# toandaominh1997/EfficientDet.Pytorch

Measured on AMD Instinct MI355X. Metric: images/sec EfficientDet-D0 512px fwd+bwd, higher is better.
Workload: dtype f32_hf16x3_bwd_bf16x3

## Files before the change

efficientdet/pytorch_amd/_lib.py:

```python
import ctypes as C
import os

import torch

HERE = os.path.dirname(os.path.abspath(__file__))
LIB_PATH = os.environ.get('EFFDET_HIP_LIB') or os.path.join(os.path.dirname(os.path.abspath(__file__)), 'libeffdet_hip.so')
MAX_SEG = 5
MAX_CONV_SEG = 10
ABI_VERSION = 11
F32, BF16, F32_BF16X3, F32_SPLIT = 0, 1, 2, 3
F32_HSPLIT = 4
ACT_NONE, ACT_RELU, ACT_SWISH, ACT_SIGMOID = 0, 1, 2, 3
RES_NONE, RES_ADD, RES_RELU_MASK, RES_SWISH_GRAD = 0, 1, 2, 3
TUNE_IGEMM_BIG, TUNE_IGEMM_BIG_MIN_M, TUNE_SPLIT_PERS, TUNE_IGEMM_KORD, TUNE_SPLIT_KORD = 0, 1, 2, 3, 4

_ERR = {-1: 'EFFDET_EINVAL', -2: 'EFFDET_ELAUNCH', -3: 'EFFDET_EUNSUPPORTED'}


class Seg(C.Structure):
    _fields_ = [('H', C.c_int), ('W', C.c_int), ('Ho', C.c_int), ('Wo', C.c_int),
                ('in_off', C.c_longlong), ('in_bstride', C.c_longlong),
                ('out_off', C.c_longlong), ('out_bstride', C.c_longlong)]


# ... 200 lines not shown
}
EMA_SIGNATURES = {
    'effdet_clip_adamw_step_ema': 'i:ppppppppiippffffffifipps',
    'effdet_clip_adamw_step_gated_ema': 'i:pppppppppiippfffffffippps',
    'effdet_ema_swap': 'i:pppppiis',
}
PLAN_SIGNATURES = {
    'effdet_dwconv_plan_info': 'i:iiiiiiiiiiiiip',
}
LIVE_SIGNATURES = {
    'effdet_live_tiles_counts': 'q:iipppp',
    'effdet_live_tiles': 'i:piiiippppps',
    'effdet_conv2d_live': 'i:ppis',
    'effdet_conv2d_wgrad_live': 'i:ppqps',
}
BOX_LOSS_SIGNATURES = {
    'effdet_box_loss_fwd': 'i:ppppppqiqiiifs',
    'effdet_box_loss_fwd_grad': 'i:ppppppqpiiiqiiifs',
    'effdet_box_loss_bwd_reg': 'i:ppppppiiiqiifs',
}
LOSS_OPTS_SIGNATURES = {
    'effdet_loss_opts_workspace_bytes': 'q:iqii',
    'effdet_loss_opts_fwd': 'i:ppppppqiqiips',
    'effdet_loss_opts_fwd_grad': 'i:ppppppqpiiiqiips',
    'effdet_loss_opts_bwd_cls': 'i:pppppiiiqiips',
    'effdet_loss_opts_bwd_reg': 'i:ppppppiiiqips',
}
ATSS_SIGNATURES = {
    'effdet_loss_atss_workspace_bytes': 'q:iqiip',
    'effdet_loss_atss_fwd': 'i:ppppppqiqiipps',
# ... 16 lines not shown
    global _lib
    if _lib is None:
        if not os.path.exists(LIB_PATH):
            raise RuntimeError(
                'libeffdet_hip.so is missing (%s). Build it with `python -m efficientdet.pytorch_amd.build` '
                '(or __graft_entry__.build()). There is no CPU fallback for this path.' % LIB_PATH)
        cand = C.CDLL(LIB_PATH)
        got = int(cand.effdet_abi_version()) if hasattr(cand, 'effdet_abi_version') else 0
        if got != ABI_VERSION:
            raise RuntimeError('%s has ABI generation %d, this binding needs %d: rebuild it (`python -m efficientdet.pytorch_amd.build`)'
                               % (LIB_PATH, got, ABI_VERSION))
        _lib = cand
        for name, sig in list(SIGNATURES.items()) + list(ADDED_SIGNATURES.items()) + list(EMA_SIGNATURES.items()) + \
                list(PLAN_SIGNATURES.items()) + list(LIVE_SIGNATURES.items()) + list(BOX_LOSS_SIGNATURES.items()) + \
                list(LOSS_OPTS_SIGNATURES.items()) + list(ATSS_SIGNATURES.items()) + list(CONV_PLAN_SIGNATURES.items()) + \
                list(WBF_SIGNATURES.items()):
            f = getattr(_lib, name, None)
            if f is not None:
                f.restype, f.argtypes = _CTYPE[sig[0]], [_CTYPE[c] for c in sig[2:]]
    return _lib


def require(*names):
    L = lib()
    missing = [n for n in names if not hasattr(L, n)]
    if missing:
        raise RuntimeError('%s does not export %s: it predates this binding, rebuild it (`python -m efficientdet.pytorch_amd.build`)'
                           % (LIB_PATH, ', '.join(missing)))
    return L


# ... 25 lines not shown
```

efficientdet/pytorch_amd/csrc/conv_igemm.hip:

```cpp
#include "common.h"
#include "../../../include/effdet_live_tiles.h"
#include "../../../include/effdet_conv_plan.h"
#include <stdlib.h>

#ifndef EFFDET_IGEMM_BIG_DEFAULT
#define EFFDET_IGEMM_BIG_DEFAULT 1
#endif

namespace {

struct SegD {
  int H, W, Ho, Wo, M, tile_start;
  long long in_off, in_bs, out_off, out_bs;
  unsigned x_bytes;
  long long w_off;
  long long sh_off;
};

struct ConvK {
  const void* x; const void* w; void* y; void* z; const void* res;
  const float* scale; const float* shift; const float* rowscale;
  const float* bc_scale; const float* bc_shift;
  int Cin, Cout, KW, stride, pad_t, pad_l;
  int ldx, ldy;
  int Kc;
  int cpt;
  int act, res_mode, out_f32, vec_ok;
  int out_split;
  int* range_flag;
  void* ysplit;
  int nseg, mtiles, ntiles;
  unsigned w_bytes;
  int kord;
  long long w_img_bytes;
  const unsigned char* live;
  int live_tile0;
  SegD seg[EFFDET_MAX_CONV_SEG];
};

constexpr int BM = 128;
typedef float f32x16 __attribute__((ext_vector_type(16)));

template <typename T> struct Mma;
template <> struct Mma<bf16_t> {
  static __device__ __forceinline__ void run(const uint4& a, const uint4& b, f32x4& c) {
    c = __builtin_amdgcn_mfma_f32_16x16x32_bf16(__builtin_bit_cast(bf16x8, a), __builtin_bit_cast(bf16x8, b), c, 0, 0, 0);
  }
};
struct MmaH {
  static __device__ __forceinline__ void run(const uint4& a, const uint4& b, f32x4& c) {
    c = __builtin_amdgcn_mfma_f32_16x16x32_f16(__builtin_bit_cast(f16x8, a), __builtin_bit_cast(f16x8, b), c, 0, 0, 0);
// ... 31 lines not shown

  const int tid = threadIdx.x;
  const int lane = tid & 63, wave = tid >> 6;
  const int wm0 = (wave / WAVES_N) * WTM, wn0 = (wave % WAVES_N) * WTN;

  int tile = xcd_remap(blockIdx.x, gridDim.x);
  if constexpr (SPLIT == 2) {
    if (p.live) {
      const int b = blockIdx.x, whole = (p.mtiles >> 3) << 3;
      if (b < whole * p.ntiles) {
        const int i = b >> 3, j = i / p.ntiles;
        tile = (j * 8 + (b & 7)) * p.ntiles + (i - j * p.ntiles);
      } else tile = b;
    }
  }
  const int mt = tile / p.ntiles, nt = tile - mt * p.ntiles;
  int si = 0;
#pragma unroll
  for (int s = 1; s < EFFDET_MAX_CONV_SEG; ++s)
    if (s < p.nseg && mt >= p.seg[s].tile_start) si = s;
  const SegD sg = p.seg[si];
  const int m_base = (mt - sg.tile_start) * BM;
  const int n_base = nt * BN;
  const int HoWo = sg.Ho * sg.Wo;

  if constexpr (SPLIT == 2) {
    if (p.live && mt >= p.live_tile0 && p.live[mt - p.live_tile0] == 0) {
      if (p.res_mode == EFFDET_RES_ADD) return;
      const int rows = min(BM, sg.M - m_base), nch = min(BN, p.Cout - n_base);
      if (p.vec_ok) {
        const int q4 = nch >> 2;
        for (int i = tid; i < rows * q4; i += NTHREADS) {
          const int row = i / q4, c = i - row * q4;
          const int m = m_base + row, bi = m / HoWo, pix = m - bi * HoWo;
          *(uint4*)((float*)p.y + sg.out_off + (long long)bi * sg.out_bs + (long long)pix * p.ldy + n_base + 4 * c) = make_uint4(0u, 0u, 0u, 0u);
        }
      } else {
        for (int i = tid; i < rows * nch; i += NTHREADS) {
          const int row = i / nch, c = i - row * nch;
          const int m = m_base + row, bi = m / HoWo, pix = m - bi * HoWo;
          ((float*)p.y)[sg.out_off + (long long)bi * sg.out_bs + (long long)pix * p.ldy + n_base + c] = 0.f;
        }
      }
      return;
    }
  }

  constexpr unsigned ES = sizeof(T);
  const long long w_img = p.w_img_bytes ? (long long)(m_base / HoWo) * p.w_img_bytes : 0ll;
  const u32x4_t rx = make_srd_raw((const T*)p.x + sg.in_off, sg.x_bytes), rw = make_srd_raw((const char*)p.w + w_img + sg.w_off, p.w_bytes);
// ... 1032 lines not shown
  k.bc_scale = p->bc_scale; k.bc_shift = p->bc_shift;
  if ((p->bc_scale != nullptr) != (p->bc_shift != nullptr)) return EFFDET_EINVAL;
  k.Cin = p->Cin; k.Cout = p->Cout; k.KW = p->KW; k.stride = p->stride; k.pad_t = p->pad_t; k.pad_l = p->pad_l;
  k.ldx = p->ldx; k.ldy = p->ldy;
  k.cpt = p->Cin / ce; k.Kc = p->KH * p->KW * k.cpt;
  k.act = p->act; k.res_mode = p->res_mode; k.out_f32 = p->out_f32; k.kord = g_tuning[EFFDET_TUNE_IGEMM_KORD];
  k.out_split = (splitfmt && !p->out_f32) ? 1 : 0;
  if (splitfmt) {
    if (g_tuning[EFFDET_TUNE_SPLIT_KORD] < 0) g_tuning[EFFDET_TUNE_SPLIT_KORD] = getenv("EFFDET_SPLIT_KORD") ? atoi(getenv("EFFDET_SPLIT_KORD")) : 1;
    const int kv = g_tuning[EFFDET_TUNE_SPLIT_KORD];
    k.kord = ((kv == 1 || (kv == 2 && p->Cout <= 64)) && k.cpt % 8 == 0) ? 1 : 0;
  }
  k.nseg = p->nseg;
  k.w_img_bytes = p->w_image_stride;
  k.live = nullptr; k.live_tile0 = 0;
  if (p->w_image_stride) {
    if (p->w_image_stride < 0 || (p->w_image_stride & 15) || p->nseg != 1 || splitfmt || (p->seg[0].Ho * p->seg[0].Wo) % BM) return EFFDET_EUNSUPPORTED;
  }
  int tiles = 0;
  bool per_seg = false;
  bool vec = (p->ldy % 4 == 0) && (p->Cout % 4 == 0);
  for (int s = 0; s < p->nseg; ++s) {
    const effdet_seg_t& g = p->seg[s];
    SegD& d = k.seg[s];
    d.H = g.H; d.W = g.W; d.Ho = g.Ho; d.Wo = g.Wo;
    d.M = p->B * g.Ho * g.Wo;
    d.tile_start = tiles;
    d.in_off = g.in_off; d.in_bs = g.in_bstride; d.out_off = g.out_off; d.out_bs = g.out_bstride;
    d.w_off = p->seg_w[s] ? (long long)((const char*)p->seg_w[s] - (const char*)p->w) : 0ll;
    d.sh_off = p->seg_shift[s] ? (long long)(p->seg_shift[s] - p->shift) : 0ll;
// ... 85 lines not shown
}

extern "C" int effdet_conv2d_live(const effdet_conv_t* p, const unsigned char* live, int live_tile0, effdet_stream_t stream) {
  ConvPlan c;
  const int id = plan_conv(p, c);
  if (id < 0) return id;
  if (live_tile0 < 0) return EFFDET_EINVAL;
  const bool plain = !p->scale && !p->shift && !p->rowscale && !p->bc_scale && !p->z && !p->y_split && p->act == EFFDET_ACT_NONE && !p->w_image_stride;
  bool no_shift = true;
  for (int s = 0; s < p->nseg; ++s) if (p->seg_shift[s]) no_shift = false;
  const bool res_ok = p->out_f32 ? (p->res_mode == EFFDET_RES_NONE || (p->res_mode == EFFDET_RES_ADD && p->res == p->y))
                                 : (p->res_mode == EFFDET_RES_NONE || p->res_mode == EFFDET_RES_RELU_MASK);
  if (live && (id == 8 || id == 9) && plain && no_shift && res_ok) { c.k.live = live; c.k.live_tile0 = live_tile0; }
  return c.launch(c, (hipStream_t)stream);
}
```

efficientdet/pytorch_amd/csrc/live_tiles.hip:

```cpp
#include "common.h"
#include "../../../include/effdet_live_tiles.h"

namespace {

struct LiveK {
  const void* dreg; unsigned char* nz; unsigned char* hd; unsigned char* l32; unsigned char* l128;
  int nlev, reg_ld, apix, ntiles;
  unsigned mask;
  long long S32, S128, P;
  int H[EFFDET_MAX_SEG], W[EFFDET_MAX_SEG], M[EFFDET_MAX_SEG];
  int pix0[EFFDET_MAX_SEG];
  int poff[EFFDET_MAX_SEG];
  int step0[EFFDET_MAX_SEG], tile0[EFFDET_MAX_SEG];
};

__global__ __launch_bounds__(256) void live_nz_kernel(const LiveK p) {
  const int sub = threadIdx.x & 15;
  const int q4 = p.reg_ld >> 2;
  for (long long g = (long long)blockIdx.x * 16 + (threadIdx.x >> 4); g < p.P; g += (long long)gridDim.x * 16) {
    int l = 0;
#pragma unroll
    for (int s = 1; s < EFFDET_MAX_SEG; ++s)
      if (s < p.nlev && g >= p.pix0[s]) l = s;
    const int m = (int)(g - p.pix0[l]);
// ... 102 lines not shown
  const int rc = live_geometry(B, nlev, H, W, k);
  if (rc != EFFDET_OK) return rc;
  k.dreg = dreg; k.nz = scratch; k.hd = scratch + k.P; k.l32 = live32; k.l128 = live128; k.reg_ld = reg_ld;
  k.mask = dtype == EFFDET_F32 ? 0x7fffffffu : 0x7fff7fffu;
  hipStream_t st = (hipStream_t)stream;
  long long g = (k.P + 63) / 64;
  if (g > 8192) g = 8192;
  hipLaunchKernelGGL(live_nz_kernel, dim3((unsigned)g), dim3(256), 0, st, k);
  EFFDET_CHECK_LAUNCH();
  hipLaunchKernelGGL(live_hdist_kernel, dim3((unsigned)((k.P + 255) / 256)), dim3(256), 0, st, k);
  EFFDET_CHECK_LAUNCH();
  hipLaunchKernelGGL(live_flags_kernel, dim3((unsigned)k.ntiles), dim3(128), 0, st, k);
  EFFDET_CHECK_LAUNCH();
  return EFFDET_OK;
}
```

efficientdet/pytorch_amd/csrc/loss.hip:

```cpp
#include "common.h"
#include "../../../include/effdet_box_loss.h"
#include "../../../include/effdet_loss_opts.h"
#include "../../../include/effdet_atss.h"

namespace {

constexpr int SS = 32;
constexpr int CLS_IT = 8;
constexpr int FG_IT = 4;

struct LossK {
  const float* cls; const float* reg; const float* anchors; const float* annots; const float* gscale;
  float* losses; int* assign; float* stat;
  float* part_reg; float* part_cls; int na, ncb;
  void* dcls; void* dreg;
  int B, nc, N; long long A;
  int dld;
  int reg_ld;
};

struct OptsK {
  float pos_iou, neg_iou; int low_quality;
  int* gtmax; float* best; int* barg;
};
// ... 185 lines not shown
  for (int n0 = 0; n0 < p.N; n0 += 64) {
    __syncthreads();
    if (threadIdx.x == 0) nvalid_s = compact_chunk(p, b, n0, ann);
    __syncthreads();
    const int c = nvalid_s;
    total_valid += c;
    if (ok) {
      for (int j = 0; j < c; ++j) {
        const float iou = assign_iou(an, aarea, ann + j * 5);
        if (iou > best) { best = iou; barg = (int)ann[j * 5 + 4]; }
      }
    }
  }
  assign_tail(p, b, a, ok, ok && total_valid > 0, best < 0.4f, best >= 0.5f, barg, an, KneeDefault{});
  if (blockIdx.x == 0 && threadIdx.x == 0) p.stat[b * SS + 3] = (float)total_valid;
}

__global__ __launch_bounds__(256) void opts_iou_kernel(const LossK p, const OptsK o) {
  const int b = blockIdx.y;
  const long long a = blockIdx.x * 256LL + threadIdx.x;
  __shared__ float ann[64 * 5];
  __shared__ int gm[64];
  __shared__ int nvalid_s;
  float best = -1.0f; int barg = -1;
  float4 an = make_float4(0, 0, 0, 0);
  const bool ok = a < p.A;
  if (ok) an = ((const float4*)p.anchors)[a];
  const float aarea = (an.z - an.x) * (an.w - an.y);
  int total_valid = 0;
  for (int n0 = 0; n0 < p.N; n0 += 64) {
// ... 634 lines not shown
  if (const int rc = check_dreg(dreg, reg_ld, dtype, A)) return rc;
  LossK k = loss_args(nullptr, reg, anchors, annots, B, A, 0, N); k.gscale = gscale; k.dreg = dreg; k.reg_ld = reg_ld;
  carve_loss(k, const_cast<void*>(workspace), B, A);
  launch(k, (hipStream_t)stream);
  EFFDET_CHECK_LAUNCH();
  return EFFDET_OK;
}

}

extern "C" long long effdet_loss_workspace_bytes(int B, long long A, int num_classes) {
  LossK k{};
  return (long long)carve_loss(k, nullptr, B, A, num_classes);
}

extern "C" long long effdet_loss_opts_workspace_bytes(int B, long long A, int num_classes, int N) {
  LossK k{}; OptsK o{};
  return (long long)carve_loss_opts(k, o, nullptr, B, A, num_classes, N);
}

extern "C" int effdet_focal_loss_fwd(const float* cls, const float* reg, const float* anchors, const float* annots,
                                     float* losses, void* workspace, long long workspace_bytes, int B, long long A,
                                     int num_classes, int N, effdet_stream_t stream) {
  LossK k = loss_args(cls, reg, anchors, annots, B, A, num_classes, N); k.losses = losses;
  return loss_forward_default(k, workspace, workspace_bytes, false, EFFDET_F32, stream);
}

extern "C" int effdet_focal_loss_fwd_grad(const float* cls, const float* reg, const float* anchors, const float* annots,
                                          float* losses, void* workspace, long long workspace_bytes, void* dcls_pix, int dld,
                                          int dtype, int B, long long A, int num_classes, int N, effdet_stream_t stream) {
// ... 117 lines not shown
```

efficientdet/pytorch_amd/efficientdet.py:

```python
import math
import os

import torch
import torch.nn as nn

from . import functional as Fn
from . import ops
from .config import (BN_EPS, DROP_CONNECT_RATE, EFFICIENTDET, MODEL_MAP, backbone_plan)
from .ops import Map


class _Holder(nn.Module):
    def forward(self, *a, **k):
        raise RuntimeError('parameter container: executed through libeffdet_hip.so, not called directly')


class _MBConvParams(_Holder):

    def __init__(self, blk):
        super().__init__()
        if blk.expand != 1:
            self._expand_conv = nn.Conv2d(blk.cin, blk.cexp, 1, bias=False)
            self._bn0 = nn.BatchNorm2d(blk.cexp, momentum=0.01, eps=BN_EPS)
        self._depthwise_conv = nn.Conv2d(blk.cexp, blk.cexp, blk.k, groups=blk.cexp, bias=False)
# ... 265 lines not shown


LOSS_FWD_GRAD = os.environ.get('EFFDET_LOSS_FWD_GRAD', '1') == '1'


class _HeadLossFn(torch.autograd.Function):

    @staticmethod
    def forward(ctx, dtype, num_classes, anchors, annots, train, box, loss, *args):
        ctx.prep, ctx.arith, ctx.box, ctx.loss = ops.get_prep(), ops.F32_ARITH_BWD, box, loss
        ctx.matcher = matcher = args[5 + len(_HEAD_KEYS)] if len(args) > 5 + len(_HEAD_KEYS) else None
        ctx.extra = len(args) - 5 - len(_HEAD_KEYS)
        p = [Map.of(t) for t in args[:5]]
        HP = dict(zip(_HEAD_KEYS, args[5:]))
        levels = [m.H * m.W * 9 for m in p] if matcher is not None else None
        cls, reg, saved = Fn.head_fwd(p, HP, num_classes, dtype, train)
        nc = num_classes
        if train and nc % 4 == 0 and LOSS_FWD_GRAD:
            dld = (9 * nc + 63) // 64 * 64
            losses, ws, dpix = ops.loss_opts_fwd_grad(cls, reg, anchors, annots, dtype, dld, split=saved[5], loss=loss, box=box,
                                                      matcher=matcher, levels=levels)
            ctx.saved = (saved, None, reg, anchors, annots, ws, dtype, dpix, dld)
        else:
            losses, ws = ops.loss_opts_fwd(cls, reg, anchors, annots, loss, box, matcher=matcher, levels=levels)
            ctx.saved = (saved, cls, reg, anchors, annots, ws, dtype, None, 0) if train else None
        return losses[0:1].clone(), losses[1:2].clone()

    @staticmethod
    def backward(ctx, gcls, greg):
        with ops.backward_scope(ctx.prep, ctx.arith):
            return _HeadLossFn._bwd(ctx, gcls, greg)
# ... 249 lines not shown
```

efficientdet/pytorch_amd/functional.py:

```python
import os

import torch

from . import ops
from .config import BN_EPS, conv_out
from .ops import ACT_NONE, ACT_RELU, ACT_SIGMOID, ACT_SWISH, RES_ADD, RES_NONE, RES_RELU_MASK, Map

DW_SAVE_Y = os.environ.get('EFFDET_DW_SAVE_Y', '0') == '1'
BIFPN_WGRAD_GROUP = os.environ.get('EFFDET_BIFPN_WGRAD_GROUP', '1') != '0'
EXPAND_Z_ONLY = os.environ.get('EFFDET_EXPAND_Z_ONLY', '1') == '1'
SE_FUSED = os.environ.get('EFFDET_SE_FUSED', '1') == '1'
DW_BWD_FUSED = os.environ.get('EFFDET_DW_BWD_FUSED', '1') == '1'
PW_BWD_FUSED = os.environ.get('EFFDET_PW_BWD_FUSED', '1') == '1'
PW_DGRAD_SE = os.environ.get('EFFDET_PW_DGRAD_SE', '1') == '1'
FUSE_EXPAND_DW = os.environ.get('EFFDET_FUSE_EXPAND_DW', '1') == '1'
FUSE_CIN = tuple(int(v) for v in os.environ.get('EFFDET_FUSE_CIN', '16,24,32').split(','))
BIFPN_F16X3_MIN_WORK = float(os.environ.get('EFFDET_BIFPN_F16X3_MIN_WORK', '1.2e8'))
GATE_IN_WEIGHTS = os.environ.get('EFFDET_GATE_IN_WEIGHTS', '1') == '1'
GATE_IN_WEIGHTS_TRAIN = os.environ.get('EFFDET_GATE_IN_WEIGHTS_TRAIN', '0') == '1'


def chunk_elems(dtype):
    return 8 if dtype == torch.bfloat16 else 4

# ... 353 lines not shown
        return torch.cuda.stream(self.s) if self.on else contextlib.nullcontext()

    def join(self):
        if self.on:
            self.main.wait_stream(self.s)
            self.on = False

    def __exit__(self, et, ev, tb):
        self.join()
        return False


HEAD_PAIR_TOWERS = os.environ.get('EFFDET_HEAD_PAIR_TOWERS', '1') == '1'
HEAD_SPLIT = os.environ.get('EFFDET_HEAD_SPLIT', '1') == '1'
HEAD_SPARSE_REG = os.environ.get('EFFDET_HEAD_SPARSE_REG', '1') == '1'
_split_ok = {}


def head_uses_split(B, sizes, Wc, dtype, arith=None):
    if not (HEAD_SPLIT and dtype == torch.float32 and (arith or ops.F32_ARITH) == 'bf16x3' and Wc % 32 == 0):
        return False
    key = (B, tuple(sizes), Wc)
    if key not in _split_ok:
        _split_ok[key] = ops.wgrad_split_supported(B, sizes, 256, 256, 256) and ops.wgrad_split_supported(B, sizes, Wc, 256, 256)
    return _split_ok[key]


def _pyramid_to_split(src_maps, B, sizes, C_, dtype, dev, bf=True, h=False):
    dst = pyramid_alloc(B, sizes, C_, dtype, dev)[1] if bf else None
    dsth = pyramid_alloc(B, sizes, C_, dtype, dev)[1] if h else None
    for i, s_ in enumerate(src_maps):
        ops.to_split2(s_.tensor(), dst[i].addr() if bf else None, dsth[i].addr() if h else None, s_.B * s_.H * s_.W * s_.C,
                      ops.range_flag(dev) if h else None)
    return dst, dsth


def head_uses_f16x3(Wc, dtype):
    return HEAD_SPLIT and dtype == torch.float32 and ops.F32_ARITH == 'f32' and ops.F32_ARITH_HEAD == 'f16x3' and Wc % 32 == 0


def head_fwd(p, HP, num_classes, dtype, train):
    dev = p[0].t.device
    B, Wc = p[0].B, p[0].C
    sizes = [(m.H, m.W) for m in p]
    A = sum(h * w for (h, w) in sizes) * 9
    split = head_uses_split(B, sizes, Wc, dtype)
    split_bwd = (not split) and train and ops.F32_ARITH_BWD == 'bf16x3' and head_uses_split(B, sizes, Wc, dtype, 'bf16x3')
    hs = (not split) and head_uses_f16x3(Wc, dtype) and (split_bwd or not train)
    pin, pin_h = p, None
    if split or split_bwd or hs:
        pin, pin_h = _pyramid_to_split(p, B, sizes, Wc, dtype, dev, bf=split or split_bwd, h=hs)
        if pin is None:
            pin = p
    acts = {'cls': [], 'reg': []}
    cls = torch.empty((B, A, num_classes), dtype=torch.float32, device=dev)
    reg = torch.empty((B, A, 4), dtype=torch.float32, device=dev)

    def tower_fwd(tower):
        cur = pin_h if hs else (p if split_bwd else pin)
        for t in range(4):
            w, b = HP[f'{tower}_convs.{t}.weight'], HP[f'{tower}_convs.{t}.bias']
            _, nxt = pyramid_alloc(B, sizes, 256, dtype, dev)
            nxs = pyramid_alloc(B, sizes, 256, dtype, dev)[1] if split_bwd else None
            ops.conv2d(cur, ops.pack_weight(w, dtype, x3=split, h3=hs), nxt, Cin=w.shape[1], Cout=256, KH=3, KW=3, pad_t=1, pad_l=1,
                       shift=b, act=ACT_RELU, split=split, ysplit=nxs, hsplit=hs)
            acts[tower].append(nxs if split_bwd else nxt); cur = nxt
        if tower == 'cls':
            ops.conv2d(cur, ops.pack_weight(HP['retina_cls.weight'], dtype, x3=split, h3=hs), head_out_maps(cls, B, sizes, num_classes),
                       Cin=256, Cout=9 * num_classes, KH=3, KW=3, pad_t=1, pad_l=1, shift=HP['retina_cls.bias'],
                       act=ACT_SIGMOID, out_f32=True, split=split, hsplit=hs)
        else:
            ops.conv2d(cur, ops.pack_weight(HP['retina_reg.weight'], dtype, x3=split, h3=hs), head_out_maps(reg, B, sizes, 4),
                       Cin=256, Cout=36, KH=3, KW=3, pad_t=1, pad_l=1, shift=HP['retina_reg.bias'], out_f32=True, split=split, hsplit=hs)
    paired = hs and HEAD_PAIR_TOWERS
    if paired:
        cur = {'cls': pin_h, 'reg': pin_h}
        for t in range(4):
            w2 = [HP[f'{tw}_convs.{t}.weight'] for tw in ('cls', 'reg')]
            b2 = [HP[f'{tw}_convs.{t}.bias'] for tw in ('cls', 'reg')]
            wp2 = [ops.pack_weight(w, dtype, h3=True) for w in w2]
            _, ya, yb = pyramid_alloc_pair(B, sizes, 256, dtype, dev)
            sa = sb = None
            if split_bwd:
                _, sa, sb = pyramid_alloc_pair(B, sizes, 256, dtype, dev)
            L5 = len(sizes)
            ops.conv2d(cur['cls'] + cur['reg'], wp2[0], ya + yb, Cin=w2[0].shape[1], Cout=256, KH=3, KW=3, pad_t=1, pad_l=1, shift=b2[0],
                       act=ACT_RELU, hsplit=True, ysplit=(sa + sb) if split_bwd else None,
                       seg_w=[wp2[0]] * L5 + [wp2[1]] * L5, seg_shift=[b2[0]] * L5 + [b2[1]] * L5)
            acts['cls'].append(sa if split_bwd else ya); acts['reg'].append(sb if split_bwd else yb)
            cur = {'cls': ya, 'reg': yb}
        ops.conv2d(cur['cls'], ops.pack_weight(HP['retina_cls.weight'], dtype, h3=True), head_out_maps(cls, B, sizes, num_classes),
                   Cin=256, Cout=9 * num_classes, KH=3, KW=3, pad_t=1, pad_l=1, shift=HP['retina_cls.bias'],
                   act=ACT_SIGMOID, out_f32=True, hsplit=True)
        ops.conv2d(cur['reg'], ops.pack_weight(HP['retina_reg.weight'], dtype, h3=True), head_out_maps(reg, B, sizes, 4),
                   Cin=256, Cout=36, KH=3, KW=3, pad_t=1, pad_l=1, shift=HP['retina_reg.bias'], out_f32=True, hsplit=True)
    else:
        with _Fork(dev, HEAD_TWO_STREAMS and ops.PROFILE is None) as fk:
            with fk.side():
                tower_fwd('reg')
            tower_fwd('cls')
    saved = (pin, acts, sizes, HP, num_classes, split or split_bwd, paired and split_bwd) if train else None
    return cls, reg, saved


def _split_rows(maps, Cfp, dtype):
    out = []
    for m in maps:
        padded = ops.pad_rows(m, Cfp) if (m.C != Cfp or m.ld != Cfp or m.bstride != m.H * m.W * Cfp or m.off) else m
        out.append(Map.of(ops.to_split(padded.tensor())))
    return out
# ... 100 lines not shown
```

efficientdet/pytorch_amd/ops.py:

```python
import ctypes as C
import os
import threading

import numpy as np
import torch

from . import _lib as L
from ._lib import (ACT_NONE, ACT_RELU, ACT_SIGMOID, ACT_SWISH, RES_ADD, RES_NONE,
                   RES_RELU_MASK, RES_SWISH_GRAD)


class LaunchProfile:

    def __init__(self):
        self.records = []

    def summary(self):
        torch.cuda.synchronize()
        out = {}
        for name, flops, e0, e1, _, nbytes in self.records:
            d = out.setdefault(name, {'launches': 0, 'flops': 0.0, 'ms': 0.0, 'bytes': 0.0})
            d['launches'] += 1; d['flops'] += flops; d['ms'] += e0.elapsed_time(e1); d['bytes'] += nbytes
        return out

# ... 324 lines not shown


def scale_pack_weight(w_oihw, gate, dtype):
    Cout, Cin = w_oihw.shape[0], w_oihw.shape[1]
    assert w_oihw.shape[2:] == (1, 1) and gate.shape[1] == Cin and gate.dtype == torch.float32 and gate.is_contiguous()
    B = gate.shape[0]
    code = _mma_dtype_code(dtype, Cin, Cout)
    out = torch.empty((B, Cout, Cin), dtype=dtype, device=gate.device)
    L.check(L.lib().effdet_scale_pack_weight(L.ptr(w_oihw.detach()), L.ptr(gate), L.ptr(out), code, B, Cout, Cin, L.stream_ptr()),
            'effdet_scale_pack_weight')
    return out, Cout * Cin * out.element_size()


def _conv_desc(xs, wp, ys, *, Cin, Cout, KH, KW, stride=1, pad_t=0, pad_l=0, scale=None, shift=None, act=ACT_NONE,
               res=None, res_mode=RES_NONE, rowscale=None, zs=None, out_f32=False, split=False, bc_scale=None, bc_shift=None,
               w_image_stride=0, ysplit=None, hsplit=False, seg_w=None, seg_shift=None, live=None, live_tile0=0):
    if isinstance(xs, Map):
        xs, ys = [xs], [ys]
        zs = [zs] if zs is not None else None
        res = [res] if res is not None else None
        ysplit = [ysplit] if ysplit is not None else None
    d = L.ConvDesc()
    x0, y0 = xs[0], ys[0]
    isx, isy = x0.t.element_size(), y0.t.element_size()
    base_x = min(x.addr() for x in xs)
    base_y = min(y.addr() for y in ys)
    d.x, d.w, d.y = base_x, wp.data_ptr(), base_y
    d.z = d.res = None
    if zs is not None:
        bz = min(z.addr() for z in zs)
        for y, z in zip(ys, zs):
# ... 16 lines not shown
        d.y_split = bs
    d.scale, d.shift, d.rowscale = (t.data_ptr() if t is not None else None for t in (scale, shift, rowscale))
    d.bc_scale, d.bc_shift = (t.data_ptr() if t is not None else None for t in (bc_scale, bc_shift))
    assert not (hsplit and (split or scale is not None))
    d.dtype, d.out_f32 = (L.F32_HSPLIT if hsplit else (L.F32_SPLIT if split else _mma_dtype_code(x0.dtype, KH * KW * Cin, Cout))), int(out_f32)
    d.B, d.Cin, d.Cout, d.KH, d.KW = x0.B, Cin, Cout, KH, KW
    d.stride, d.pad_t, d.pad_l = stride, pad_t, pad_l
    d.ldx, d.ldy = x0.ld, y0.ld
    d.act, d.res_mode = act, res_mode
    d.w_image_stride = int(w_image_stride)
    _segs(d, xs, ys, base_x, base_y, isx, isy)
    if live is not None:
        assert live.dtype == torch.uint8 and live.is_contiguous()
        ntile = sum((y.B * y.H * y.W + 127) // 128 for y in ys)
        assert 0 <= live_tile0 <= ntile and live.numel() == ntile - live_tile0, (live.numel(), ntile, live_tile0)
    return d, xs, ys


def conv2d(xs, wp, ys, *, Cin, Cout, KH, KW, stride=1, pad_t=0, pad_l=0, scale=None, shift=None, act=ACT_NONE,
           res=None, res_mode=RES_NONE, rowscale=None, zs=None, out_f32=False, split=False, bc_scale=None, bc_shift=None,
           w_image_stride=0, ysplit=None, hsplit=False, seg_w=None, seg_shift=None, live=None, live_tile0=0):
    d, xs, ys = _conv_desc(xs, wp, ys, Cin=Cin, Cout=Cout, KH=KH, KW=KW, stride=stride, pad_t=pad_t, pad_l=pad_l, scale=scale, shift=shift,
                           act=act, res=res, res_mode=res_mode, rowscale=rowscale, zs=zs, out_f32=out_f32, split=split, bc_scale=bc_scale,
                           bc_shift=bc_shift, w_image_stride=w_image_stride, ysplit=ysplit, hsplit=hsplit, seg_w=seg_w, seg_shift=seg_shift,
                           live=live, live_tile0=live_tile0)
    x0, y0 = xs[0], ys[0]
    isx, isy = x0.t.element_size(), y0.t.element_size()
    flops = 2.0 * KH * KW * Cin * Cout * sum(y.B * y.H * y.W for y in ys)
    nbytes = isx * Cin * sum(x.B * x.H * x.W for x in xs) + wp.numel() * wp.element_size() + \
        (4 if out_f32 else isy) * Cout * sum(y.B * y.H * y.W for y in ys) * (1 + (zs is not None) + (ysplit is not None) + (res is not None))
    if live is not None:
        run = lambda: L.check(L.require('effdet_conv2d_live').effdet_conv2d_live(C.byref(d), live.data_ptr(), int(live_tile0), L.stream_ptr()),
                              'effdet_conv2d_live')
    else:
        run = lambda: L.check(L.lib().effdet_conv2d(C.byref(d), L.stream_ptr()), 'effdet_conv2d')
    _timed(_igemm_symbol(x0.dtype, d) if PROFILE is not None else '', flops, run,
           'k%d s%d Cin%d Cout%d M%d' % (KH, stride, Cin, Cout, sum(y.B * y.H * y.W for y in ys)), nbytes=float(nbytes))


def conv2d_plan_info(xs, wp, ys, **kw):
    d, _, _ = _conv_desc(xs, wp, ys, **kw)
    info = L.ConvPlanInfo()
    rc = int(L.require('effdet_conv2d_plan_info').effdet_conv2d_plan_info(C.byref(d), C.byref(info)))
    if rc < 0:
        L.check(rc, 'effdet_conv2d_plan_info')
    out = {n: int(getattr(info, n)) for n, _ in L.ConvPlanInfo._fields_ if n != 'reserved'}
    out['form'] = L.CONV_FORMS[out['form']]
    out['persistent'], out['m32'] = bool(out['persistent']), bool(out['m32'])
    return out


def _wgrad_desc(xs, dzs, dw, dbias, Cin, Cout, KH, KW, stride, pad_t, pad_l, want_bias, split, image_splits):
# ... 183 lines not shown
def live_tiles(dreg, B, sizes, reg_ld, split):
    lib_ = L.require(*L.LIVE_SIGNATURES)
    n = len(sizes)
    Hs, Ws = (C.c_int * n)(*[h for h, _ in sizes]), (C.c_int * n)(*[w for _, w in sizes])
    steps, tiles = C.c_longlong(), C.c_longlong()
    pixels = int(lib_.effdet_live_tiles_counts(B, n, Hs, Ws, C.byref(steps), C.byref(tiles)))
    if pixels < 0:
        L.check(pixels, 'effdet_live_tiles_counts')
    assert dreg.is_contiguous() and dreg.element_size() == 4 and dreg.numel() == pixels * reg_ld
    S, T, R = steps.value, tiles.value, L.LIVE_RADII
    buf = torch.empty(R * S + R * T + 2 * pixels, dtype=torch.uint8, device=dreg.device)
    l32, l128, scratch = buf[:R * S].view(R, S), buf[R * S:R * (S + T)].view(R, T), buf[R * (S + T):]
    L.check(lib_.effdet_live_tiles(dreg.data_ptr(), L.F32_SPLIT if split else L.F32, reg_ld, B, n, Hs, Ws, scratch.data_ptr(),
                                   l32.data_ptr(), l128.data_ptr(), L.stream_ptr()), 'effdet_live_tiles')
    return l32, l128


def to_split(t):
    assert t.dtype == torch.float32 and t.is_contiguous() and t.numel() % 32 == 0
    out = torch.empty_like(t)
    L.check(L.lib().effdet_to_split(L.ptr(t), L.ptr(out), t.numel(), L.stream_ptr()), 'effdet_to_split')
    return out


def to_split2(src, dst_split, dst_hsplit, n, flag=None):
    if dst_hsplit is None:
        L.check(L.lib().effdet_to_split(L.ptr(src), dst_split, n, L.stream_ptr()), 'effdet_to_split')
    else:
        L.check(L.lib().effdet_to_split2(L.ptr(src), dst_split, dst_hsplit, n, L.ptr(flag), L.stream_ptr()), 'effdet_to_split2')

# ... 1106 lines not shown
```

Measured before the change: 1259.

## Skip forward regression-head conv tiles whose receptive field has no positive anchors

Adds a kernel that builds a per-pixel map of positive anchors (IoU ≥ 0.5 with any annotation) and dilates it into per-tile needed flags using the existing live-tile machinery. The forward regression tower convs and the regression output conv then zero out tiles that cannot influence any positive-anchor regression output instead of computing them. This removes forward GEMM work in the reg head during training, at the cost of extra IoU-map and flag kernels per step. It relies on the regression loss only reading positive anchors, so the zeroed regression outputs in skipped tiles are never used.

```diff
diff --git a/efficientdet/pytorch_amd/_lib.py b/efficientdet/pytorch_amd/_lib.py
--- a/efficientdet/pytorch_amd/_lib.py
+++ b/efficientdet/pytorch_amd/_lib.py
@@ -238,6 +238,11 @@
     'effdet_conv2d_live': 'i:ppis',
     'effdet_conv2d_wgrad_live': 'i:ppqps',
 }
+NEEDED_SIGNATURES = {
+    'effdet_positive_pixel_map': 'i:ppiqiippps',
+    'effdet_live_tiles_from_map': 'i:piippppps',
+    'effdet_conv2d_needed': 'i:ppis',
+}
 BOX_LOSS_SIGNATURES = {
     'effdet_box_loss_fwd': 'i:ppppppqiqiiifs',
     'effdet_box_loss_fwd_grad': 'i:ppppppqpiiiqiiifs',
@@ -284,7 +289,7 @@
         for name, sig in list(SIGNATURES.items()) + list(ADDED_SIGNATURES.items()) + list(EMA_SIGNATURES.items()) + \
                 list(PLAN_SIGNATURES.items()) + list(LIVE_SIGNATURES.items()) + list(BOX_LOSS_SIGNATURES.items()) + \
                 list(LOSS_OPTS_SIGNATURES.items()) + list(ATSS_SIGNATURES.items()) + list(CONV_PLAN_SIGNATURES.items()) + \
-                list(WBF_SIGNATURES.items()):
+                list(WBF_SIGNATURES.items()) + list(NEEDED_SIGNATURES.items()):
             f = getattr(_lib, name, None)
             if f is not None:
                 f.restype, f.argtypes = _CTYPE[sig[0]], [_CTYPE[c] for c in sig[2:]]
diff --git a/efficientdet/pytorch_amd/csrc/conv_igemm.hip b/efficientdet/pytorch_amd/csrc/conv_igemm.hip
--- a/efficientdet/pytorch_amd/csrc/conv_igemm.hip
+++ b/efficientdet/pytorch_amd/csrc/conv_igemm.hip
@@ -1,5 +1,6 @@
 #include "common.h"
 #include "../../../include/effdet_live_tiles.h"
+#include "../../../include/effdet_needed_tiles.h"
 #include "../../../include/effdet_conv_plan.h"
 #include <stdlib.h>
 
@@ -35,6 +36,8 @@
   long long w_img_bytes;
   const unsigned char* live;
   int live_tile0;
+  const unsigned char* needed;
+  int needed_tile0;
   SegD seg[EFFDET_MAX_CONV_SEG];
 };
 
@@ -96,6 +99,15 @@
       } else tile = b;
     }
   }
+  if constexpr (SPLIT == 3) {
+    if (p.needed) {
+      const int b = blockIdx.x, whole = (p.mtiles >> 3) << 3;
+      if (b < whole * p.ntiles) {
+        const int i = b >> 3, j = i / p.ntiles;
+        tile = (j * 8 + (b & 7)) * p.ntiles + (i - j * p.ntiles);
+      } else tile = b;
+    }
+  }
   const int mt = tile / p.ntiles, nt = tile - mt * p.ntiles;
   int si = 0;
 #pragma unroll
@@ -116,6 +128,29 @@
           const int row = i / q4, c = i - row * q4;
           const int m = m_base + row, bi = m / HoWo, pix = m - bi * HoWo;
           *(uint4*)((float*)p.y + sg.out_off + (long long)bi * sg.out_bs + (long long)pix * p.ldy + n_base + 4 * c) = make_uint4(0u, 0u, 0u, 0u);
+        }
+      } else {
+        for (int i = tid; i < rows * nch; i += NTHREADS) {
+          const int row = i / nch, c = i - row * nch;
+          const int m = m_base + row, bi = m / HoWo, pix = m - bi * HoWo;
+          ((float*)p.y)[sg.out_off + (long long)bi * sg.out_bs + (long long)pix * p.ldy + n_base + c] = 0.f;
+        }
+      }
+      return;
+    }
+  }
+
+  if constexpr (SPLIT == 3) {
+    if (p.needed && mt >= p.needed_tile0 && p.needed[mt - p.needed_tile0] == 0) {
+      const int rows = min(BM, sg.M - m_base), nch = min(BN, p.Cout - n_base);
+      if (p.vec_ok) {
+        const int q4 = nch >> 2;
+        for (int i = tid; i < rows * q4; i += NTHREADS) {
+          const int row = i / q4, c = i - row * q4;
+          const int m = m_base + row, bi = m / HoWo, pix = m - bi * HoWo;
+          const long long o = sg.out_off + (long long)bi * sg.out_bs + (long long)pix * p.ldy + n_base + 4 * c;
+          *(uint4*)((float*)p.y + o) = make_uint4(0u, 0u, 0u, 0u);
+          if (p.ysplit) *(uint4*)((float*)p.ysplit + o) = make_uint4(0u, 0u, 0u, 0u);
         }
       } else {
         for (int i = tid; i < rows * nch; i += NTHREADS) {
@@ -1178,6 +1213,7 @@
   k.nseg = p->nseg;
   k.w_img_bytes = p->w_image_stride;
   k.live = nullptr; k.live_tile0 = 0;
+  k.needed = nullptr; k.needed_tile0 = 0;
   if (p->w_image_stride) {
     if (p->w_image_stride < 0 || (p->w_image_stride & 15) || p->nseg != 1 || splitfmt || (p->seg[0].Ho * p->seg[0].Wo) % BM) return EFFDET_EUNSUPPORTED;
   }
@@ -1293,3 +1329,12 @@
   if (live && (id == 8 || id == 9) && plain && no_shift && res_ok) { c.k.live = live; c.k.live_tile0 = live_tile0; }
   return c.launch(c, (hipStream_t)stream);
 }
+
+extern "C" int effdet_conv2d_needed(const effdet_conv_t* p, const unsigned char* needed, int needed_tile0, effdet_stream_t stream) {
+  ConvPlan c;
+  const int id = plan_conv(p, c);
+  if (id < 0) return id;
+  if (needed_tile0 < 0) return EFFDET_EINVAL;
+  if (needed && (id == 30 || id == 31) && (c.k.vec_ok || (p->out_f32 && !p->y_split))) { c.k.needed = needed; c.k.needed_tile0 = needed_tile0; }
+  return c.launch(c, (hipStream_t)stream);
+}
diff --git a/efficientdet/pytorch_amd/csrc/live_tiles.hip b/efficientdet/pytorch_amd/csrc/live_tiles.hip
--- a/efficientdet/pytorch_amd/csrc/live_tiles.hip
+++ b/efficientdet/pytorch_amd/csrc/live_tiles.hip
@@ -1,5 +1,6 @@
 #include "common.h"
 #include "../../../include/effdet_live_tiles.h"
+#include "../../../include/effdet_needed_tiles.h"
 
 namespace {
 
@@ -140,3 +141,18 @@
   EFFDET_CHECK_LAUNCH();
   return EFFDET_OK;
 }
+
+extern "C" int effdet_live_tiles_from_map(const unsigned char* map, int B, int nlev, const int* H, const int* W, unsigned char* scratch,
+                                          unsigned char* live32, unsigned char* live128, effdet_stream_t stream) {
+  if (!map || !scratch || !live32 || !live128) return EFFDET_EINVAL;
+  LiveK k;
+  const int rc = live_geometry(B, nlev, H, W, k);
+  if (rc != EFFDET_OK) return rc;
+  k.dreg = nullptr; k.nz = const_cast<unsigned char*>(map); k.hd = scratch + k.P; k.l32 = live32; k.l128 = live128; k.reg_ld = 0; k.mask = 0u;
+  hipStream_t st = (hipStream_t)stream;
+  hipLaunchKernelGGL(live_hdist_kernel, dim3((unsigned)((k.P + 255) / 256)), dim3(256), 0, st, k);
+  EFFDET_CHECK_LAUNCH();
+  hipLaunchKernelGGL(live_flags_kernel, dim3((unsigned)k.ntiles), dim3(128), 0, st, k);
+  EFFDET_CHECK_LAUNCH();
+  return EFFDET_OK;
+}
diff --git a/efficientdet/pytorch_amd/csrc/loss.hip b/efficientdet/pytorch_amd/csrc/loss.hip
--- a/efficientdet/pytorch_amd/csrc/loss.hip
+++ b/efficientdet/pytorch_amd/csrc/loss.hip
@@ -2,6 +2,7 @@
 #include "../../../include/effdet_box_loss.h"
 #include "../../../include/effdet_loss_opts.h"
 #include "../../../include/effdet_atss.h"
+#include "../../../include/effdet_needed_tiles.h"
 
 namespace {
 
@@ -223,6 +224,52 @@
   }
   assign_tail(p, b, a, ok, ok && total_valid > 0, best < 0.4f, best >= 0.5f, barg, an, KneeDefault{});
   if (blockIdx.x == 0 && threadIdx.x == 0) p.stat[b * SS + 3] = (float)total_valid;
+}
+
+struct PosMapK {
+  unsigned char* map; int nlev, apix;
+  int hw[EFFDET_MAX_SEG], poff[EFFDET_MAX_SEG], pix0[EFFDET_MAX_SEG];
+};
+
+__global__ __launch_bounds__(256) void loss_pos_map_kernel(const LossK p, const PosMapK g) {
+  const int b = blockIdx.y;
+  const int q = blockIdx.x * 256 + threadIdx.x;
+  __shared__ float ann[64 * 5];
+  __shared__ int nvalid_s;
+  const bool ok = q < g.apix;
+  float4 an[9]; float aarea[9], best[9];
+#pragma unroll
+  for (int k = 0; k < 9; ++k) {
+    an[k] = ok ? ((const float4*)p.anchors)[(long long)q * 9 + k] : make_float4(0, 0, 0, 0);
+    aarea[k] = (an[k].z - an[k].x) * (an[k].w - an[k].y);
+    best[k] = -1.0f;
+  }
+  int total_valid = 0;
+  for (int n0 = 0; n0 < p.N; n0 += 64) {
+    __syncthreads();
+    if (threadIdx.x == 0) nvalid_s = compact_chunk(p, b, n0, ann);
+    __syncthreads();
+    const int c = nvalid_s;
+    total_valid += c;
+    if (ok) {
+      for (int j = 0; j < c; ++j) {
+#pragma unroll
+        for (int k = 0; k < 9; ++k) {
+          const float iou = assign_iou(an[k], aarea[k], ann + j * 5);
+          if (iou > best[k]) best[k] = iou;
+        }
+      }
+    }
+  }
+  if (!ok) return;
+  bool pos = false;
+#pragma unroll
+  for (int k = 0; k < 9; ++k) pos = pos || (best[k] >= 0.5f);
+  int l = 0;
+#pragma unroll
+  for (int s = 1; s < EFFDET_MAX_SEG; ++s)
+    if (s < g.nlev && q >= g.poff[s]) l = s;
+  g.map[(long long)g.pix0[l] + (long long)b * g.hw[l] + (q - g.poff[l])] = (pos && total_valid > 0) ? 1 : 0;
 }
 
 __global__ __launch_bounds__(256) void opts_iou_kernel(const LossK p, const OptsK o) {
@@ -887,6 +934,30 @@
   return (long long)carve_loss(k, nullptr, B, A, num_classes);
 }
 
+extern "C" int effdet_positive_pixel_map(const float* anchors, const float* annots, int B, long long A, int N, int nlev, const int* H,
+                                         const int* W, unsigned char* map, effdet_stream_t stream) {
+  if (!anchors || !annots || !map || !H || !W) return EFFDET_EINVAL;
+  if (B < 1 || B > 65535 || N < 1 || nlev < 1 || nlev > EFFDET_MAX_SEG) return EFFDET_EINVAL;
+  PosMapK g{}; g.map = map; g.nlev = nlev;
+  long long apix = 0, P = 0;
+  for (int l = 0; l < nlev; ++l) {
+    if (H[l] < 1 || W[l] < 1) return EFFDET_EINVAL;
+    apix += (long long)H[l] * W[l];
+  }
+  if (A != 9 * apix) return EFFDET_EINVAL;
+  if (apix * B >= 0x40000000LL) return EFFDET_EUNSUPPORTED;
+  g.apix = (int)apix; apix = 0;
+  for (int l = 0; l < nlev; ++l) {
+    const long long hw = (long long)H[l] * W[l];
+    g.hw[l] = (int)hw; g.poff[l] = (int)apix; g.pix0[l] = (int)P;
+    apix += hw; P += hw * B;
+  }
+  const LossK k = loss_args(nullptr, nullptr, anchors, annots, B, A, 0, N);
+  hipLaunchKernelGGL(loss_pos_map_kernel, dim3((unsigned)((apix + 255) / 256), B), dim3(256), 0, (hipStream_t)stream, k, g);
+  EFFDET_CHECK_LAUNCH();
+  return EFFDET_OK;
+}
+
 extern "C" long long effdet_loss_opts_workspace_bytes(int B, long long A, int num_classes, int N) {
   LossK k{}; OptsK o{};
   return (long long)carve_loss_opts(k, o, nullptr, B, A, num_classes, N);
diff --git a/efficientdet/pytorch_amd/efficientdet.py b/efficientdet/pytorch_amd/efficientdet.py
--- a/efficientdet/pytorch_amd/efficientdet.py
+++ b/efficientdet/pytorch_amd/efficientdet.py
@@ -303,7 +303,10 @@
         p = [Map.of(t) for t in args[:5]]
         HP = dict(zip(_HEAD_KEYS, args[5:]))
         levels = [m.H * m.W * 9 for m in p] if matcher is not None else None
-        cls, reg, saved = Fn.head_fwd(p, HP, num_classes, dtype, train)
+        need = None
+        if matcher is None and loss is None and Fn.head_fwd_takes_needed(p, dtype, train):
+            need = ops.needed_tiles(anchors, annots, p[0].B, [(m.H, m.W) for m in p])
+        cls, reg, saved = Fn.head_fwd(p, HP, num_classes, dtype, train, reg_needed=need)
         nc = num_classes
         if train and nc % 4 == 0 and LOSS_FWD_GRAD:
             dld = (9 * nc + 63) // 64 * 64
diff --git a/efficientdet/pytorch_amd/functional.py b/efficientdet/pytorch_amd/functional.py
--- a/efficientdet/pytorch_amd/functional.py
+++ b/efficientdet/pytorch_amd/functional.py
@@ -391,6 +391,7 @@
 HEAD_PAIR_TOWERS = os.environ.get('EFFDET_HEAD_PAIR_TOWERS', '1') == '1'
 HEAD_SPLIT = os.environ.get('EFFDET_HEAD_SPLIT', '1') == '1'
 HEAD_SPARSE_REG = os.environ.get('EFFDET_HEAD_SPARSE_REG', '1') == '1'
+HEAD_SPARSE_REG_FWD = os.environ.get('EFFDET_HEAD_SPARSE_REG_FWD', '1') == '1'
 _split_ok = {}
 
 
@@ -416,14 +417,30 @@
     return HEAD_SPLIT and dtype == torch.float32 and ops.F32_ARITH == 'f32' and ops.F32_ARITH_HEAD == 'f16x3' and Wc % 32 == 0
 
 
-def head_fwd(p, HP, num_classes, dtype, train):
+def _head_forms(B, sizes, Wc, dtype, train):
+    split = head_uses_split(B, sizes, Wc, dtype)
+    split_bwd = (not split) and train and ops.F32_ARITH_BWD == 'bf16x3' and head_uses_split(B, sizes, Wc, dtype, 'bf16x3')
+    hs = (not split) and head_uses_f16x3(Wc, dtype) and (split_bwd or not train)
+    return split, split_bwd, hs
+
+
+def head_fwd_takes_needed(p, dtype, train):
+    _, split_bwd, hs = _head_forms(p[0].B, [(m.H, m.W) for m in p], p[0].C, dtype, train)
+    return bool(HEAD_SPARSE_REG_FWD and train and hs and split_bwd)
+
+
+def head_fwd(p, HP, num_classes, dtype, train, reg_needed=None):
     dev = p[0].t.device
     B, Wc = p[0].B, p[0].C
     sizes = [(m.H, m.W) for m in p]
     A = sum(h * w for (h, w) in sizes) * 9
-    split = head_uses_split(B, sizes, Wc, dtype)
-    split_bwd = (not split) and train and ops.F32_ARITH_BWD == 'bf16x3' and head_uses_split(B, sizes, Wc, dtype, 'bf16x3')
-    hs = (not split) and head_uses_f16x3(Wc, dtype) and (split_bwd or not train)
+    split, split_bwd, hs = _head_forms(B, sizes, Wc, dtype, train)
+    if not (hs and split_bwd):
+        reg_needed = None
+    ntile = sum((B * h * w + 127) // 128 for (h, w) in sizes)
+
+    def need(r):
+        return reg_needed[r] if reg_needed is not None else None
     pin, pin_h = p, None
     if split or split_bwd or hs:
         pin, pin_h = _pyramid_to_split(p, B, sizes, Wc, dtype, dev, bf=split or split_bwd, h=hs)
@@ -440,7 +457,7 @@
             _, nxt = pyramid_alloc(B, sizes, 256, dtype, dev)
             nxs = pyramid_alloc(B, sizes, 256, dtype, dev)[1] if split_bwd else None
             ops.conv2d(cur, ops.pack_weight(w, dtype, x3=split, h3=hs), nxt, Cin=w.shape[1], Cout=256, KH=3, KW=3, pad_t=1, pad_l=1,
-                       shift=b, act=ACT_RELU, split=split, ysplit=nxs, hsplit=hs)
+                       shift=b, act=ACT_RELU, split=split, ysplit=nxs, hsplit=hs, needed=need(4 - t) if tower == 'reg' else None)
             acts[tower].append(nxs if split_bwd else nxt); cur = nxt
         if tower == 'cls':
             ops.conv2d(cur, ops.pack_weight(HP['retina_cls.weight'], dtype, x3=split, h3=hs), head_out_maps(cls, B, sizes, num_classes),
@@ -448,7 +465,8 @@
                        act=ACT_SIGMOID, out_f32=True, split=split, hsplit=hs)
         else:
             ops.conv2d(cur, ops.pack_weight(HP['retina_reg.weight'], dtype, x3=split, h3=hs), head_out_maps(reg, B, sizes, 4),
-                       Cin=256, Cout=36, KH=3, KW=3, pad_t=1, pad_l=1, shift=HP['retina_reg.bias'], out_f32=True, split=split, hsplit=hs)
+                       Cin=256, Cout=36, KH=3, KW=3, pad_t=1, pad_l=1, shift=HP['retina_reg.bias'], out_f32=True, split=split, hsplit=hs,
+                       needed=need(0))
     paired = hs and HEAD_PAIR_TOWERS
     if paired:
         cur = {'cls': pin_h, 'reg': pin_h}
@@ -463,14 +481,15 @@
             L5 = len(sizes)
             ops.conv2d(cur['cls'] + cur['reg'], wp2[0], ya + yb, Cin=w2[0].shape[1], Cout=256, KH=3, KW=3, pad_t=1, pad_l=1, shift=b2[0],
                        act=ACT_RELU, hsplit=True, ysplit=(sa + sb) if split_bwd else None,
-                       seg_w=[wp2[0]] * L5 + [wp2[1]] * L5, seg_shift=[b2[0]] * L5 + [b2[1]] * L5)
+                       seg_w=[wp2[0]] * L5 + [wp2[1]] * L5, seg_shift=[b2[0]] * L5 + [b2[1]] * L5,
+                       needed=need(4 - t), needed_tile0=ntile if reg_needed is not None else 0)
             acts['cls'].append(sa if split_bwd else ya); acts['reg'].append(sb if split_bwd else yb)
             cur = {'cls': ya, 'reg': yb}
         ops.conv2d(cur['cls'], ops.pack_weight(HP['retina_cls.weight'], dtype, h3=True), head_out_maps(cls, B, sizes, num_classes),
                    Cin=256, Cout=9 * num_classes, KH=3, KW=3, pad_t=1, pad_l=1, shift=HP['retina_cls.bias'],
                    act=ACT_SIGMOID, out_f32=True, hsplit=True)
         ops.conv2d(cur['reg'], ops.pack_weight(HP['retina_reg.weight'], dtype, h3=True), head_out_maps(reg, B, sizes, 4),
-                   Cin=256, Cout=36, KH=3, KW=3, pad_t=1, pad_l=1, shift=HP['retina_reg.bias'], out_f32=True, hsplit=True)
+                   Cin=256, Cout=36, KH=3, KW=3, pad_t=1, pad_l=1, shift=HP['retina_reg.bias'], out_f32=True, hsplit=True, needed=need(0))
     else:
         with _Fork(dev, HEAD_TWO_STREAMS and ops.PROFILE is None) as fk:
             with fk.side():
diff --git a/efficientdet/pytorch_amd/ops.py b/efficientdet/pytorch_amd/ops.py
--- a/efficientdet/pytorch_amd/ops.py
+++ b/efficientdet/pytorch_amd/ops.py
@@ -362,7 +362,7 @@
 
 def _conv_desc(xs, wp, ys, *, Cin, Cout, KH, KW, stride=1, pad_t=0, pad_l=0, scale=None, shift=None, act=ACT_NONE,
                res=None, res_mode=RES_NONE, rowscale=None, zs=None, out_f32=False, split=False, bc_scale=None, bc_shift=None,
-               w_image_stride=0, ysplit=None, hsplit=False, seg_w=None, seg_shift=None, live=None, live_tile0=0):
+               w_image_stride=0, ysplit=None, hsplit=False, seg_w=None, seg_shift=None, live=None, live_tile0=0, needed=None, needed_tile0=0):
     if isinstance(xs, Map):
         xs, ys = [xs], [ys]
         zs = [zs] if zs is not None else None
@@ -409,16 +409,20 @@
         assert live.dtype == torch.uint8 and live.is_contiguous()
         ntile = sum((y.B * y.H * y.W + 127) // 128 for y in ys)
         assert 0 <= live_tile0 <= ntile and live.numel() == ntile - live_tile0, (live.numel(), ntile, live_tile0)
+    if needed is not None:
+        assert live is None and needed.dtype == torch.uint8 and needed.is_contiguous()
+        ntile = sum((y.B * y.H * y.W + 127) // 128 for y in ys)
+        assert 0 <= needed_tile0 <= ntile and needed.numel() == ntile - needed_tile0, (needed.numel(), ntile, needed_tile0)
     return d, xs, ys
 
 
 def conv2d(xs, wp, ys, *, Cin, Cout, KH, KW, stride=1, pad_t=0, pad_l=0, scale=None, shift=None, act=ACT_NONE,
            res=None, res_mode=RES_NONE, rowscale=None, zs=None, out_f32=False, split=False, bc_scale=None, bc_shift=None,
-           w_image_stride=0, ysplit=None, hsplit=False, seg_w=None, seg_shift=None, live=None, live_tile0=0):
+           w_image_stride=0, ysplit=None, hsplit=False, seg_w=None, seg_shift=None, live=None, live_tile0=0, needed=None, needed_tile0=0):
     d, xs, ys = _conv_desc(xs, wp, ys, Cin=Cin, Cout=Cout, KH=KH, KW=KW, stride=stride, pad_t=pad_t, pad_l=pad_l, scale=scale, shift=shift,
                            act=act, res=res, res_mode=res_mode, rowscale=rowscale, zs=zs, out_f32=out_f32, split=split, bc_scale=bc_scale,
                            bc_shift=bc_shift, w_image_stride=w_image_stride, ysplit=ysplit, hsplit=hsplit, seg_w=seg_w, seg_shift=seg_shift,
-                           live=live, live_tile0=live_tile0)
+                           live=live, live_tile0=live_tile0, needed=needed, needed_tile0=needed_tile0)
     x0, y0 = xs[0], ys[0]
     isx, isy = x0.t.element_size(), y0.t.element_size()
     flops = 2.0 * KH * KW * Cin * Cout * sum(y.B * y.H * y.W for y in ys)
@@ -427,10 +431,17 @@
     if live is not None:
         run = lambda: L.check(L.require('effdet_conv2d_live').effdet_conv2d_live(C.byref(d), live.data_ptr(), int(live_tile0), L.stream_ptr()),
                               'effdet_conv2d_live')
+    elif needed is not None:
+        NEEDED_LAUNCHES[0] += 1
+        run = lambda: L.check(L.require('effdet_conv2d_needed').effdet_conv2d_needed(C.byref(d), needed.data_ptr(), int(needed_tile0),
+                                                                                     L.stream_ptr()), 'effdet_conv2d_needed')
     else:
         run = lambda: L.check(L.lib().effdet_conv2d(C.byref(d), L.stream_ptr()), 'effdet_conv2d')
     _timed(_igemm_symbol(x0.dtype, d) if PROFILE is not None else '', flops, run,
            'k%d s%d Cin%d Cout%d M%d' % (KH, stride, Cin, Cout, sum(y.B * y.H * y.W for y in ys)), nbytes=float(nbytes))
+
+
+NEEDED_LAUNCHES = [0]
 
 
 def conv2d_plan_info(xs, wp, ys, **kw):
@@ -644,6 +655,42 @@
     L.check(lib_.effdet_live_tiles(dreg.data_ptr(), L.F32_SPLIT if split else L.F32, reg_ld, B, n, Hs, Ws, scratch.data_ptr(),
                                    l32.data_ptr(), l128.data_ptr(), L.stream_ptr()), 'effdet_live_tiles')
     return l32, l128
+
+
+def _level_arrays(sizes):
+    n = len(sizes)
+    return n, (C.c_int * n)(*[h for h, _ in sizes]), (C.c_int * n)(*[w for _, w in sizes])
+
+
+def positive_pixel_map(anc, annots, sizes):
+    B, N = annots.shape[0], annots.shape[1]
+    A = anc.numel() // 4
+    n, Hs, Ws = _level_arrays(sizes)
+    assert anc.dtype == torch.float32 and anc.is_contiguous() and annots.dtype == torch.float32 and annots.is_contiguous()
+    out = torch.empty(B * sum(h * w for h, w in sizes), dtype=torch.uint8, device=annots.device)
+    L.check(L.require('effdet_positive_pixel_map').effdet_positive_pixel_map(L.ptr(anc), L.ptr(annots), B, A, N, n, Hs, Ws, out.data_ptr(),
+                                                                             L.stream_ptr()), 'effdet_positive_pixel_map')
+    return out
+
+
+def live_tiles_from_map(pixmap, B, sizes):
+    lib_ = L.require('effdet_live_tiles_counts', 'effdet_live_tiles_from_map')
+    n, Hs, Ws = _level_arrays(sizes)
+    steps, tiles = C.c_longlong(), C.c_longlong()
+    pixels = int(lib_.effdet_live_tiles_counts(B, n, Hs, Ws, C.byref(steps), C.byref(tiles)))
+    if pixels < 0:
+        L.check(pixels, 'effdet_live_tiles_counts')
+    assert pixmap.dtype == torch.uint8 and pixmap.is_contiguous() and pixmap.numel() == pixels
+    S, T, R = steps.value, tiles.value, L.LIVE_RADII
+    buf = torch.empty(R * S + R * T + 2 * pixels, dtype=torch.uint8, device=pixmap.device)
+    l32, l128, scratch = buf[:R * S].view(R, S), buf[R * S:R * (S + T)].view(R, T), buf[R * (S + T):]
+    L.check(lib_.effdet_live_tiles_from_map(pixmap.data_ptr(), B, n, Hs, Ws, scratch.data_ptr(), l32.data_ptr(), l128.data_ptr(),
+                                            L.stream_ptr()), 'effdet_live_tiles_from_map')
+    return l32, l128
+
+
+def needed_tiles(anc, annots, B, sizes):
+    return live_tiles_from_map(positive_pixel_map(anc, annots, sizes), B, sizes)[1]
 
 
 def to_split(t):
diff --git a/include/effdet_needed_tiles.h b/include/effdet_needed_tiles.h
--- /dev/null
+++ b/include/effdet_needed_tiles.h
@@ -0,0 +1,19 @@
+#ifndef EFFDET_NEEDED_TILES_H
+#define EFFDET_NEEDED_TILES_H
+#include "effdet_live_tiles.h"
+#ifdef __cplusplus
+extern "C" {
+#endif
+
+int effdet_positive_pixel_map(const float* anchors, const float* annots, int B, long long A, int N, int nlev, const int* H,
+                              const int* W, unsigned char* map, effdet_stream_t stream);
+
+int effdet_live_tiles_from_map(const unsigned char* map, int B, int nlev, const int* H, const int* W, unsigned char* scratch,
+                               unsigned char* live32, unsigned char* live128, effdet_stream_t stream);
+
+int effdet_conv2d_needed(const effdet_conv_t* p, const unsigned char* needed, int needed_tile0, effdet_stream_t stream);
+
+#ifdef __cplusplus
+}
+#endif
+#endif
```

Measured after the change: 1341 (median of 6 runs). 6.5% higher.
